# haliphinx/TCE-RVOS

Measured on AMD Instinct MI355X. Metric: clips/s (T=5, 360×640, Swin-T) at 1/2/4/8 MI355X; mask IoU vs ref, higher is better.
Workload: dtype f32 (3xf16-split MFMA, f32 accumulate); 1 GPU; swin_t_p4w7 T=5 360x640 + 32-token text, B=1 clip per forward, flags --with_box_refine --binary --f_token 8 --qtrans (BASELINE config 2); clips_in_flight_per_gpu=1, clips_per_forward=1, same_clip_in_group=False, ranks_per_gpu=1, parallelism=clip-sharded x1

## Files before the change

### include/tce_rvos_debug.h

```cpp
#ifndef TCE_RVOS_DEBUG_H
#define TCE_RVOS_DEBUG_H
#include <stdint.h>
#ifdef __cplusplus
extern "C" {
#endif
int tce_gemm_force_tile(int32_t tile);
int tce_debug_set_stamp_buffer(long long* dev_buf);
int tce_debug_set_epilogue(int32_t lds_staged);
int tce_debug_ffn_set_stamp_buffer(long long* dev_buf);
int tce_debug_ffn_set_half(int32_t mode);
int tce_debug_msda_set_lds(int32_t on);
int tce_debug_window_attn_set_mfma(int32_t on);
int tce_debug_mha_set_split(int32_t on);
int tce_debug_msda_set_fewq(int32_t on);
int tce_debug_conv3x3_set_waves(int32_t waves);
int tce_debug_conv3x3_set_pieces(int32_t pieces);
#ifdef __cplusplus
}
#endif
#endif
```

### tce-rvos_amd/_lib.py

```python
import ctypes as C
import os

HERE = os.path.dirname(os.path.abspath(__file__))
LIB_PATH = os.environ.get("TCE_LIB") or os.path.join(HERE, "lib", "libtce_rvos.so")

c_f = C.c_void_p
i32, i64, f32 = C.c_int32, C.c_int64, C.c_float


class GemmArgs(C.Structure):
    _fields_ = [("A", c_f), ("A2", c_f), ("W", c_f), ("bias", c_f), ("res", c_f), ("C", c_f),
                ("M", i32), ("N", i32), ("K", i32),
                ("lda", i32), ("lda2", i32), ("ldw", i32), ("ldc", i32), ("ldres", i32),
                ("act", i32), ("res_mode", i32), ("batch", i32),
                ("sA", i64), ("sA2", i64), ("sW", i64), ("sBias", i64), ("sC", i64), ("sRes", i64),
                ("conv", i32), ("T", i32), ("H", i32), ("Wd", i32), ("Cin", i32), ("Ho", i32), ("Wo", i32),
                ("kh", i32), ("kw", i32), ("stride", i32), ("pad", i32)]


class RowLinArgs(C.Structure):
    _fields_ = [("x", c_f), ("a2", c_f), ("packed", c_f), ("bias", c_f), ("res", c_f), ("out", c_f),
                ("g_in", c_f), ("be_in", c_f), ("g_out", c_f), ("be_out", c_f),
                ("ldx", i64), ("lda2", i64), ("ldres", i64), ("ldo", i64),
                ("sX", i64), ("sA2", i64), ("sRes", i64), ("sOut", i64),
# ... 67 lines not shown
    "tce_mha_ws_bytes": (i64, [i32, i32, i32]),
    "tce_mha_ws_f32": (i32, [c_f, c_f, c_f, c_f, c_f, i32, i32, i32, i32, i32, i32, i32, i32, i64, i64, i64, i64, c_f, f32, c_f]),
    "tce_ms_deform_attn_forward_f32": (i32, [c_f, c_f, c_f, c_f, c_f, c_f, i32, i32, i32, i32, i32, i32, i32, c_f]),
    "tce_ms_deform_attn_backward_f32": (i32, [c_f, c_f, c_f, c_f, c_f, c_f, c_f, c_f, c_f, i32, i32, i32, i32, i32, i32, i32, c_f]),
    "tce_msda_fused_f32": (i32, [c_f, c_f, c_f, c_f, C.POINTER(i32), i32, i32, i32, i32, i32, i32, i32, i32, c_f]),
    "tce_msda_fused_valid_f32": (i32, [c_f, c_f, c_f, c_f, C.POINTER(i32), C.POINTER(i32), i32, i32, i32, i32, i32, i32, i32,
                                       i32, c_f]),
    "tce_msda_fewq_raw_f32": (i32, [c_f, c_f, c_f, c_f, c_f, c_f, C.POINTER(i32), C.POINTER(i32), i32, i32, i32, i32, i32, i32, i32,
                                    i32, c_f]),
    "tce_contrastive_f32": (i32, [c_f, c_f, c_f, c_f, i32, i32, i32, i32, c_f]),
    "tce_pos_sine2d_f32": (i32, [c_f, c_f, i32, i32, i32, i32, c_f]),
    "tce_pos_sine2d_valid_f32": (i32, [c_f, c_f, i32, i32, i32, i32, i32, i32, c_f]),
    "tce_resize_nearest_f32": (i32, [c_f, c_f, c_f, i32, i32, i32, i32, i32, i32, c_f]),
    "tce_resize_bilinear_f32": (i32, [c_f, c_f, c_f, i32, i32, i32, i32, i32, i32, c_f]),
    "tce_resize_bilinear_ln_f32": (i32, [c_f, c_f, c_f, c_f, f32, c_f, i32, i32, i32, i32, i32, i32, c_f]),
    "tce_add_f32": (i32, [c_f, c_f, c_f, i64, i64, c_f]),
    "tce_tile_f32": (i32, [c_f, c_f, i64, i64, c_f]),
    "tce_sigmoid_f32": (i32, [c_f, c_f, i64, c_f]),
    "tce_copy_segments": (i32, [C.POINTER(CopySeg), i32, c_f]),
    "tce_box_refine_f32": (i32, [c_f, c_f, c_f, i32, i32, c_f]),
    "tce_mask_pack_f32": (i32, [c_f, c_f, c_f, i32, i32, i32, i32, c_f]),
    "tce_mask_tail_f32": (i32, [c_f, c_f, c_f, i32, c_f, i32, i32, i32, i32, i32, f32, f32, i32, c_f]),
    "tce_select_masks_u8": (i32, [c_f, c_f, c_f, c_f, i32, i32, i32, i32, i32, i32, i32, f32, c_f]),
    "tce_embed_ln_f32": (i32, [c_f, c_f, c_f, c_f, c_f, c_f, c_f, c_f, i32, i32, f32, i32, c_f]),
    "tce_mha_small64_f32": (i32, [c_f, c_f, i32, i32, f32, c_f]),
    "tce_mha_small64_seqs_f32": (i32, [c_f, i32, c_f, c_f, i32, i32, i32, f32, c_f]),
    "tce_embed_ln_seqs_f32": (i32, [c_f, c_f, c_f, c_f, c_f, c_f, c_f, i32, i32, i32, f32, i32, c_f]),
    "tce_mha_small64_lens_f32": (i32, [c_f, i32, c_f, c_f, i32, i32, i32, f32, c_f, c_f]),
    "tce_caption_lens_f32": (i32, [c_f, i32, i32, i32, i32, c_f, c_f, c_f, c_f]),
    "tce_tanh_f32": (i32, [c_f, c_f, i64, c_f]),
    "tce_ffn_packed_bytes": (i64, [i32, i32]),
    "tce_ffn_pack_f32": (i32, [c_f, c_f, c_f, c_f, i32, i32, c_f]),
    "tce_ffn_fused_f32": (i32, [c_f, i64, c_f, c_f, c_f, c_f, f32, c_f, c_f, f32, c_f, i64, i32, i32, i32, i32, c_f]),
    "tce_ffn_split_ws_floats": (i64, [i32, i32, i32, i32]),
    "tce_ffn_split_counters": (i32, [i32, i32, i32, i32]),
    "tce_ffn_set_wg_cap": (i32, [i32]),
    "tce_ffn_capped_grid": (i32, [i32, i32, i32, C.POINTER(i32)]),
    "tce_ffn_fused_split_f32": (i32, [c_f, i64, c_f, c_f, c_f, c_f, f32, c_f, c_f, f32, c_f, i64, i32, i32, i32, i32, c_f, i64, c_f, i32, c_f]),
    "tce_xattn_prepare_f32": (i32, [c_f, c_f, c_f, c_f, c_f, c_f, c_f, i32, i32, i32, c_f]),
    "tce_ffn_pack_batched_f32": (i32, [c_f, c_f, c_f, c_f, i32, i32, i32, c_f]),
    "tce_xattn_fused_f32": (i32, [C.POINTER(XattnArgs), c_f]),
    "tce_xattn_ffn_fused_f32": (i32, [C.POINTER(XattnArgs), C.POINTER(XattnFfnArgs), c_f]),
    "tce_ffn_pack_chain_f32": (i32, [c_f, c_f, c_f, c_f, i32, i32, c_f]),
    "tce_xattn_pack_f32": (i32, [c_f, c_f, c_f, c_f, c_f, i32, i32, i32, c_f]),
    "tce_xattn_prepare_lens_f32": (i32, [c_f, c_f, c_f, c_f, c_f, c_f, c_f, i32, i32, i32, c_f, c_f]),
    "tce_xattn_pack_lens_f32": (i32, [c_f, c_f, c_f, c_f, c_f, i32, i32, i32, c_f, c_f]),
    "tce_rowlin_packed_bytes": (i64, [i32, i32]),
    "tce_rowlin_pack_f32": (i32, [c_f, i64, c_f, i32, i32, c_f]),
    "tce_rowlin_f32": (i32, [C.POINTER(RowLinArgs), c_f]),
    "tce_conv3x3_packed_bytes": (i64, [i32, i32]),
    "tce_conv3x3_pack_f32": (i32, [c_f, c_f, i32, i32, c_f]),
    "tce_conv3x3_f32": (i32, [c_f, i64, c_f, c_f, c_f, i64, i32, i32, i32, i32, i32, c_f]),
    "tce_conv3x3_split_ws_floats": (i64, [i32, i32, i32]),
    "tce_conv3x3_split_pieces": (i32, [i32, i32, i32]),
    "tce_conv3x3_split_kstep": (i32, [i32, i32]),
    "tce_conv3x3_split_f32": (i32, [c_f, i64, c_f, c_f, c_f, i64, i32, i32, i32, i32, i32, c_f, i64, c_f]),
    "tce_fewrow_linear_f32": (i32, [C.POINTER(FewRowArgs), c_f]),
    "tce_thin_linear_splits": (i32, [i32, i32, i32]),
    "tce_thin_partials_f32": (i32, [c_f, i64, i32, c_f, i32, c_f, i64, c_f, i32, i32, i32, c_f]),
    "tce_splitk_reduce_f32": (i32, [c_f, i32, i32, i32, c_f, i32, c_f, i32, i32, c_f, i32, c_f, c_f, f32, c_f]),
    "tce_mha_small64_splits_f32": (i32, [c_f, i32, c_f, c_f, i32, i32, f32, c_f]),
    "tce_swin_attn_packed_bytes": (i64, [i32]),
    "tce_swin_attn_pack_f32": (i32, [c_f, c_f, c_f, i32, c_f]),
    "tce_swin_attn_fused_f32": (i32, [c_f, i64, c_f, c_f, c_f, c_f, c_f, c_f, f32, c_f, i64, i32, i32, i32, i32, i32, c_f]),
    "tce_graph_begin": (i32, [c_f]),
    "tce_graph_end": (i32, [c_f, C.POINTER(C.c_void_p)]),
    "tce_graph_launch": (i32, [C.c_void_p, c_f]),
    "tce_graph_destroy": (i32, [C.c_void_p]),
    "tce_graph_group": (i32, [C.POINTER(C.c_void_p), i32, C.POINTER(C.c_void_p)]),
}

DEBUG_SIGNATURES = {
    "tce_gemm_force_tile": (i32, [i32]),
    "tce_debug_set_stamp_buffer": (i32, [c_f]),
    "tce_debug_set_epilogue": (i32, [i32]),
    "tce_debug_ffn_set_stamp_buffer": (i32, [c_f]),
    "tce_debug_ffn_set_half": (i32, [i32]),
    "tce_debug_msda_set_lds": (i32, [i32]),
    "tce_debug_window_attn_set_mfma": (i32, [i32]),
    "tce_debug_mha_set_split": (i32, [i32]),
    "tce_debug_msda_set_fewq": (i32, [i32]),
    "tce_debug_conv3x3_set_waves": (i32, [i32]),
    "tce_debug_conv3x3_set_pieces": (i32, [i32]),
}

VIDEO_SIGNATURES = {
    "tce_label_objects_u8": (i32, [C.POINTER(LabelObj), i32, c_f, c_f, i32, i32, i32, i32, i32, i32, i32, f32, f32, c_f]),
}

A2D_GROUP_MAX = 16
EVAL_SIGNATURES = {
    "tce_a2d_masks_u8": (i32, [c_f, c_f, i32, i32, i32, i32, i32, i32, i32, f32, c_f]),
    "tce_rle_ws_bytes": (i64, [i32, i32, i32]),
    "tce_rle_counts_u32": (i32, [c_f, c_f, c_f, c_f, i32, i32, i32, c_f]),
    "tce_a2d_group_masks_u8": (i32, [C.POINTER(A2dGroupSample), i32, i32, i32, i32, f32, c_f]),
}

SCORE_SIGNATURES = {
    "tce_jf_ws_bytes": (i64, [i32, i32, i32, i32, i32]),
    "tce_jf_counts_i32": (i32, [c_f, c_f, c_f, c_f, i32, i32, i32, i32, i32, c_f]),
    "tce_rle_decode_ws_bytes": (i64, [i32, i32, i32, i32]),
    "tce_rle_decode_u8": (i32, [c_f, c_f, c_f, c_f, i32, i32, i32, i32, c_f]),
    "tce_mask_overlap_ws_bytes": (i64, [i32, i32, i32]),
    "tce_mask_overlap_i32": (i32, [c_f, c_f, c_f, c_f, i32, i32, i32, c_f]),
}

PNG_SIGNATURES = {
    "tce_png_stream_bound": (i64, [i32, i32, i32]),
    "tce_png_ws_bytes": (i64, [i32, i32, i32, i32]),
    "tce_png_deflate_u8": (i32, [c_f, c_f, c_f, c_f, i32, i32, i32, i32, i32, c_f]),
    "tce_png_deflate_dyn_u8": (i32, [c_f, c_f, c_f, c_f, i32, i32, i32, i32, i32, c_f]),
}

HEADERS = {"tce_rvos.h": SIGNATURES, "tce_rvos_debug.h": DEBUG_SIGNATURES, "tce_rvos_video.h": VIDEO_SIGNATURES,
           "tce_rvos_eval.h": EVAL_SIGNATURES, "tce_rvos_score.h": SCORE_SIGNATURES, "tce_rvos_png.h": PNG_SIGNATURES}

_LIB = None


class TceError(RuntimeError):
    pass


def lib():
    global _LIB
    if _LIB is None:
        if not os.path.exists(LIB_PATH):
            raise TceError(f"{LIB_PATH} not found: build the HIP extension first "
                           f"(python -c 'import __graft_entry__ as g; g.build()'); there is no fallback path")
        hwq = os.environ.get("GPU_MAX_HW_QUEUES")
        if hwq not in (None, "", "4"):
            import warnings
            warnings.warn(f"tce_rvos_amd: GPU_MAX_HW_QUEUES={hwq} is set; the HIP runtime's default (4) is the only value this "
                          f"launch program runs well with (1-3 crash the runtime, 5-16 double the clip time)", RuntimeWarning)
        l = C.CDLL(LIB_PATH)
        for name, (res, args) in [kv for table in HEADERS.values() for kv in table.items()]:
            fn = getattr(l, name)
            fn.restype, fn.argtypes = res, args
        _LIB = l
    return _LIB


def lib_raw():
    l = lib()
    return l.__dict__.get("_real", l)


def check(status, what=""):
    if status != 0:
        msg = lib().tce_last_error().decode(errors="replace")
        raise TceError(f"{what} failed ({status}): {msg}")
```

### tce-rvos_amd/csrc/rowlin.hip

```cpp
#include "common.h"
#include "gemm_epilogue.h"
#include "frag.h"
#include "tiles.h"
#include "../../include/tce_rvos.h"

namespace {

static __device__ long long* g_ffn_stamps = nullptr;

struct LinArgs {
  const float *x, *a2;
  const unsigned char* wpk;
  const float *bias, *res;
  float* out;
  const float *g_in, *be_in, *g_out, *be_out;
  long long ldx, lda2, ldres, ldo;
  long long sX, sA2, sRes, sOut;
  int M, N, a2_rows, act, res_mode;
  float eps_in, eps_out;
  int* range_flag;
  int single;
};

template <int K, bool ROW, bool SINGLE>
// ... 64 lines not shown
        fl[q] = *reinterpret_cast<const h16x8*>(st + (2 * q + 1) * PIECE);
      }
#pragma unroll
    for (int s = 0; s < KH; ++s) {
      if (s + 2 < KH) {
        fh[(s + 2) % 3] = *reinterpret_cast<const h16x8*>(st + (2 * s + 4) * PIECE);
        fl[(s + 2) % 3] = *reinterpret_cast<const h16x8*>(st + (2 * s + 5) * PIECE);
      }
      if (s < SLOTS) dma_half(s);
      __builtin_amdgcn_sched_barrier(0);
      if (!single) {
        acc = __builtin_amdgcn_mfma_f32_32x32x16_f16(fh[s % 3], xl[S0 + s], acc, 0, 0, 0);
        acc = __builtin_amdgcn_mfma_f32_32x32x16_f16(fl[s % 3], xh[S0 + s], acc, 0, 0, 0);
      }
      acc = __builtin_amdgcn_mfma_f32_32x32x16_f16(fh[s % 3], xh[S0 + s], acc, 0, 0, 0);
      __builtin_amdgcn_sched_barrier(0);
    }
    dma_next();
    cstage = cstage == 2 ? 0 : cstage + 1;
  };
  auto act_tile = [&](f32x16& acc) {
    if (p.act == 1) {
#pragma unroll
      for (int i = 0; i < 16; ++i) acc[i] = fmaxf(acc[i], 0.f);
    } else if (p.act == 2) {
#pragma unroll
      for (int i = 0; i < 16; ++i) acc[i] = tce_gelu(acc[i]);
    }
  };
  auto finish_tile = [&](f32x16& acc, const BiasTile& bt, const ResTile& rt) {
    const ResTile none = {};
    const BiasTile nob = {};
    if (p.res_mode == 0 || p.act != 0) {
      tile_bias_res<0>(acc, bt, none, wt, lane);
      act_tile(acc);
      if (p.res_mode == 1) tile_bias_res<1>(acc, nob, rt, wt, lane);
      else if (p.res_mode == 2) tile_bias_res<2>(acc, nob, rt, wt, lane);
    } else if (p.res_mode == 1) {
      tile_bias_res<1>(acc, bt, rt, wt, lane);
    } else {
      tile_bias_res<2>(acc, bt, rt, wt, lane);
    }
  };
  auto tile_mma = [&](f32x16& acc, const bool stores_follow) {
#pragma unroll
    for (int i = 0; i < 16; ++i) acc[i] = 0.f;
    half_mma(std::integral_constant<int, 0>{}, acc);
    asm volatile("s_waitcnt vmcnt(%0)" ::"n"(SLOTS) : "memory");
    __syncthreads();
    half_mma(std::integral_constant<int, 1>{}, acc);
    (void)stores_follow;
  };

  if (ROW) {
    f32x16 oacc[NTR];
#pragma unroll
    for (int t = 0; t < NTR; ++t) {
      tile_mma(oacc[t], false);
      asm volatile("s_waitcnt vmcnt(%0)" ::"n"(SLOTS) : "memory");
      __syncthreads();
    }
    {
      ResTile rt[NTR];
      if (p.res_mode != 0) {
#pragma unroll
        for (int t = 0; t < NTR; ++t) rt[t] = tile_res_load(res, p.ldres, m0, p.M, 32 * t, lane);
      }
#pragma unroll
      for (int t = 0; t < NTR; ++t) finish_tile(oacc[t], tile_bias_load(p.bias, 32 * t, lane), rt[t]);
    }
    if (p.g_out) rows_layernorm<NTR>(oacc, p.g_out, p.be_out, p.eps_out, hf);
#pragma unroll
    for (int t = 0; t < NTR; ++t) tile_store(oacc[t], out, p.ldo, m0, p.M, 32 * t, wt, lane, amax);
  } else {
    for (int t = t_begin; t < t_end; ++t) {
      ResTile rt = {};
      if (p.res_mode != 0) rt = tile_res_load(res, p.ldres, m0, p.M, 32 * t, lane);
      const BiasTile bt = tile_bias_load(p.bias, 32 * t, lane);
      f32x16 acc;
      tile_mma(acc, true);
      asm volatile("s_waitcnt vmcnt(%0)" ::"n"(SLOTS) : "memory");
      __syncthreads();
      finish_tile(acc, bt, rt);
      tile_store(acc, out, p.ldo, m0, p.M, 32 * t, wt, lane, amax);
    }
  }
  asm volatile("s_waitcnt vmcnt(0)" ::: "memory");
  tce_range_report(p.range_flag, amax);
  if (stamps) {
    stamps[2] = (long long)__builtin_amdgcn_s_memtime();
    stamps[3] = (long long)__builtin_amdgcn_s_memtime();
    stamps[5] = (long long)__builtin_amdgcn_s_memrealtime();
  }
}

__global__ void __launch_bounds__(256) rowlin_pack_kernel(const float* __restrict__ W, unsigned char* __restrict__ out,
                                                          const int N, const int K, const long long ldw,
                                                          const long long units, const int single) {
  const long long u = (long long)blockIdx.x * 256 + threadIdx.x;
  if (u >= units) return;
  const int KH = K / 32, HP = (2 * KH + 3) / 4 * 4;
  const int lane = (int)(u & 63);
  const long long pg = u >> 6;
  const int piece = (int)(pg % HP);
  const long long hb = pg / HP;
  const int t = (int)(hb >> 1), h = (int)(hb & 1);
  const int r = lane & 31, hf = lane >> 5, s = h * KH + (piece >> 1);
  u32x4 o = {0u, 0u, 0u, 0u};
  const int n = 32 * t + r;
  if (piece < 2 * KH && n < N) {
    float v[8];
#pragma unroll
    for (int j = 0; j < 8; ++j) v[j] = W[(long long)n * ldw + 16 * s + 8 * hf + j];
    const HL f = split8(v, single);
    o = __builtin_bit_cast(u32x4, (piece & 1) ? f.lo : f.hi);
  }
  reinterpret_cast<u32x4*>(out)[u] = o;
}

inline bool rowlin_shape_ok(int N, int K) {
  return (K == 96 || K == 128 || K == 192 || K == 256 || K == 384 || K == 512) && N > 0 && N % 32 == 0;
}
inline long long rowlin_units(int N, int K) {
  const int HP = (2 * (K / 32) + 3) / 4 * 4;
  return (long long)(2 * (N / 32) + 2) * HP * 64;
}

template <int K>
void rowlin_launch(const LinArgs& a, int batch, bool row, hipStream_t s) {
  const int rb = tce_cdiv(a.M, 128) * batch, ntiles = a.N / 32;
  int nz = 1;
  if (!row && K > 256) {
    nz = 256 / (rb > 0 ? rb : 1);
    if (nz > ntiles / 2) nz = ntiles / 2;
    if (nz < 1) nz = 1;
  } else if (!row) {
    while (nz < ntiles && rb * nz < 160 && ntiles / (nz * 2) >= 2) nz *= 2;
  }
  const dim3 grid(tce_cdiv(a.M, 128), batch, nz), block(256);
  if constexpr (K <= 384) {
    if (row) {
      if (a.single) hipLaunchKernelGGL((rowlin_kernel<K, true, true>), grid, block, 0, s, a);
      else hipLaunchKernelGGL((rowlin_kernel<K, true, false>), grid, block, 0, s, a);
      return;
    }
  }
  if (a.single) hipLaunchKernelGGL((rowlin_kernel<K, false, true>), grid, block, 0, s, a);
  else hipLaunchKernelGGL((rowlin_kernel<K, false, false>), grid, block, 0, s, a);
}

}

int tce_rowlin_set_stamps(long long* dev_buf) {
  return hipMemcpyToSymbol(HIP_SYMBOL(g_ffn_stamps), &dev_buf, sizeof(dev_buf)) == hipSuccess ? 0 : -1;
}

extern "C" int64_t tce_rowlin_packed_bytes(int32_t N, int32_t K) { return rowlin_shape_ok(N, K) ? rowlin_units(N, K) * 16 : -1; }

extern "C" int tce_rowlin_pack_f32(const float* W, int64_t ldw, void* packed, int32_t N, int32_t K, tceStream stream) {
  TCE_CHECK_ARG(rowlin_shape_ok(N, K), "tce_rowlin_pack_f32: unsupported shape N=%d K=%d (K in 96/128/192/256/384/512, N %% 32 == 0)", N, K);
  TCE_CHECK_ARG(W && packed && tce_aligned16(packed) && ldw >= K, "tce_rowlin_pack_f32: null / misaligned pointer or ldw < K");
  const long long units = rowlin_units(N, K);
  hipLaunchKernelGGL(rowlin_pack_kernel, dim3(tce_cdiv(units, 256)), dim3(256), 0, (hipStream_t)stream, W,
                     (unsigned char*)packed, N, K, (long long)ldw, units, tce_gemm_single_pass());
  TCE_CHECK_LAUNCH("tce_rowlin_pack_f32");
  return TCE_OK;
}

extern "C" int tce_rowlin_f32(const tceRowLinArgs* args, tceStream stream) {
  TCE_CHECK_ARG(args != nullptr, "tce_rowlin_f32: null args");
  const tceRowLinArgs& q = *args;
  TCE_CHECK_ARG(rowlin_shape_ok(q.N, q.K), "tce_rowlin_f32: unsupported shape N=%d K=%d", q.N, q.K);
  TCE_CHECK_ARG(q.M > 0 && q.x && q.packed && q.out, "tce_rowlin_f32: null pointer or M <= 0");
  TCE_CHECK_ARG(q.act >= 0 && q.act <= 2 && q.res_mode >= 0 && q.res_mode <= 2, "tce_rowlin_f32: bad act / res_mode");
  TCE_CHECK_ARG(q.res_mode == 0 || q.res, "tce_rowlin_f32: res_mode set without res");
  TCE_CHECK_ARG(q.ldx >= q.K && q.ldx % 4 == 0 && q.ldo >= q.N && q.ldo % 4 == 0 && (!q.res || (q.ldres >= q.N && q.ldres % 4 == 0)) &&
                    (!q.a2 || (q.lda2 >= q.K && q.lda2 % 4 == 0)),
                "tce_rowlin_f32: bad row pitch");
  TCE_CHECK_ARG(q.sX % 4 == 0 && q.sA2 % 4 == 0 && q.sRes % 4 == 0 && q.sOut % 4 == 0, "tce_rowlin_f32: batch strides must be multiples of 4 floats");
  TCE_CHECK_ARG(tce_aligned16(q.x) && tce_aligned16(q.out) && tce_aligned16(q.packed) && (!q.a2 || tce_aligned16(q.a2)) &&
                    (!q.res || tce_aligned16(q.res)) && (!q.bias || tce_aligned16(q.bias)),
                "tce_rowlin_f32: pointers must be 16-byte aligned");
  TCE_CHECK_ARG((!q.g_in || (q.be_in && tce_aligned16(q.g_in) && tce_aligned16(q.be_in))) &&
                    (!q.g_out || (q.be_out && tce_aligned16(q.g_out) && tce_aligned16(q.be_out))),
                "tce_rowlin_f32: LayerNorm gamma/beta must come in pairs, 16-byte aligned");
  TCE_CHECK_ARG(!q.g_out || (q.N == 256 && q.K <= 384), "tce_rowlin_f32: the output LayerNorm is built for N = 256, K <= 384");
  LinArgs a;
  a.x = q.x; a.a2 = q.a2; a.wpk = (const unsigned char*)q.packed; a.bias = q.bias; a.res = q.res; a.out = q.out;
  a.g_in = q.g_in; a.be_in = q.be_in; a.g_out = q.g_out; a.be_out = q.be_out;
  a.ldx = q.ldx; a.lda2 = q.lda2; a.ldres = q.ldres; a.ldo = q.ldo;
  a.sX = q.sX; a.sA2 = q.sA2; a.sRes = q.sRes; a.sOut = q.sOut;
  a.M = q.M; a.N = q.N; a.a2_rows = q.a2_rows; a.act = q.act; a.res_mode = q.res_mode;
  a.eps_in = q.eps_in; a.eps_out = q.eps_out; a.range_flag = tce_range_flag(); a.single = tce_gemm_single_pass();
  const int batch = q.batch > 0 ? q.batch : 1;
  const bool row = q.g_out != nullptr;
  hipStream_t s = (hipStream_t)stream;
  if (q.K == 512) rowlin_launch<512>(a, batch, row, s);
  else if (q.K == 384) rowlin_launch<384>(a, batch, row, s);
  else if (q.K == 256) rowlin_launch<256>(a, batch, row, s);
  else if (q.K == 192) rowlin_launch<192>(a, batch, row, s);
  else if (q.K == 128) rowlin_launch<128>(a, batch, row, s);
  else rowlin_launch<96>(a, batch, row, s);
  TCE_CHECK_LAUNCH("tce_rowlin_f32");
  return TCE_OK;
}
```

### tce-rvos_amd/ops.py

```python
import ctypes as C

import os
import threading

import torch

from ._lib import GemmArgs, check, lib

ACT_NONE, ACT_RELU, ACT_GELU, ACT_RELU_AFTER_RES = 0, 1, 2, 3
RES_NONE, RES_ADD, RES_MUL = 0, 1, 2


class Arena:

    ALIGN = 256
    FLAGS = 1 << 14

    def __init__(self, device, nbytes):
        self.device = torch.device(device)
        self.buf = torch.empty(int(nbytes), dtype=torch.uint8, device=self.device)
        self.off = 0
        self.peak = 0
        self.flags = torch.zeros(self.FLAGS, dtype=torch.int32, device=self.device)
        self.flag_off = 0
# ... 1170 lines not shown
            check(lib().tce_ffn_fused_split_f32(x.data_ptr(), ldx, packed.data_ptr(), b2.data_ptr(), gi, bi, eps_in, go, bo, eps_out,
                                                out.data_ptr(), ldo, M, Cn, Hd, act, ws.data_ptr(), ws.numel(), cnt.data_ptr(),
                                                cnt.numel(), _stream()), "tce_ffn_fused_split_f32")
            return
        check(lib().tce_ffn_fused_f32(x.data_ptr(), ldx, packed.data_ptr(), b2.data_ptr(), gi, bi, eps_in, go, bo, eps_out,
                                      out.data_ptr(), ldo, M, Cn, Hd, act, _stream()), "tce_ffn_fused_f32")
    if GEMM_PROFILE is None:
        go_()
        return out
    e0, e1 = torch.cuda.Event(enable_timing=True), torch.cuda.Event(enable_timing=True)
    e0.record()
    go_()
    e1.record()
    GEMM_PROFILE.append((f"ffn_fused_kernel<{Cn}", False, 4.0 * M * Cn * Hd, e0, e1))
    return out


class Routes:
    def __init__(self):
        self.rowlin = {}
        self.conv3 = {}
        self.keep = []

    def clear(self):
        self.rowlin.clear()
        self.conv3.clear()
        del self.keep[:]


DEFAULT_ROUTES = Routes()
_ROUTES = DEFAULT_ROUTES


class routes:

    def __init__(self, r):
        self.r, self.prev = r, None

    def __enter__(self):
        global _ROUTES
        self.prev, _ROUTES = _ROUTES, (self.r if self.r is not None else DEFAULT_ROUTES)
        return self

    def __exit__(self, *exc):
        global _ROUTES
        _ROUTES = self.prev
        return False


def current_routes():
    return _ROUTES


ROWLIN_MIN_ROWS = int(os.environ.get("TCE_ROWLIN_MIN_ROWS", 12000))
ROWLIN384_MAX_ROWS = int(os.environ.get("TCE_ROWLIN384_MAX_ROWS", 12000))
ROWLIN_K = (96, 128, 192, 256) + ((384,) if os.environ.get("TCE_ROWLIN_K384", "1") != "0" else ()) \
    + ((512,) if os.environ.get("TCE_ROWLIN_K512", "1") != "0" else ())


def rowlin_pack(w, N=None, K=None, ldw=None):
    _chk(w, "w")
    N = w.shape[0] if N is None else N
    K = w.shape[1] if K is None else K
    ldw = w.stride(0) if ldw is None else ldw
    nbytes = lib().tce_rowlin_packed_bytes(N, K)
    if nbytes < 0:
        raise ValueError(f"rowlin_pack: unsupported shape N={N} K={K}")
    out = torch.empty(nbytes, dtype=torch.uint8, device=w.device)
    check(lib().tce_rowlin_pack_f32(w.data_ptr(), ldw, out.data_ptr(), N, K, _stream()), "tce_rowlin_pack_f32")
    return out


def rowlin_register(w, table=None):
    if w.dim() != 2 or w.stride(1) != 1 or w.shape[1] not in ROWLIN_K or w.shape[0] % 32 or not w.is_cuda:
        return None
    r = _ROUTES if table is None else table
    key = (w.data_ptr(), w.shape[0], w.shape[1], w.stride(0), get_gemm_mode())
    if key not in r.rowlin:
        r.rowlin[key] = rowlin_pack(w)
        r.keep.append(w)
    return r.rowlin[key]


def rowlin(x, pk, out, M, N, K, ldx, ldo, bias=None, a2=None, lda2=0, a2_rows=0, act=ACT_NONE, res=None, ldres=0,
           res_mode=RES_NONE, ln_in=None, ln_out=None, eps_in=1e-5, eps_out=1e-5, batch=1, sX=0, sA2=0, sRes=0, sOut=0):
    from ._lib import RowLinArgs
    q = RowLinArgs()
    q.x, q.packed, q.out = x.data_ptr(), pk.data_ptr(), out.data_ptr()
    q.M, q.N, q.K, q.batch = M, N, K, batch
    q.ldx, q.ldo = ldx, ldo
    if a2 is not None:
        q.a2, q.lda2, q.a2_rows = a2.data_ptr(), lda2, a2_rows
    if bias is not None:
        q.bias = bias.data_ptr()
    if res_mode != RES_NONE:
        q.res, q.ldres = res.data_ptr(), ldres
    if ln_in is not None:
        q.g_in, q.be_in = ln_in[0].data_ptr(), ln_in[1].data_ptr()
    if ln_out is not None:
        q.g_out, q.be_out = ln_out[0].data_ptr(), ln_out[1].data_ptr()
    q.act, q.res_mode, q.eps_in, q.eps_out = act, res_mode, eps_in, eps_out
    q.sX, q.sA2, q.sRes, q.sOut = sX, sA2, sRes, sOut

    def go():
        check(lib().tce_rowlin_f32(C.byref(q), _stream()), "tce_rowlin_f32")
    if GEMM_PROFILE is None:
        go()
        return out
    e0, e1 = torch.cuda.Event(enable_timing=True), torch.cuda.Event(enable_timing=True)
    e0.record()
    go()
    e1.record()
    GEMM_PROFILE.append((f"rowlin_kernel<{K}", False, 2.0 * M * N * K * batch, e0, e1))
    return out


CONV3_MIN_PIXELS = int(os.environ.get("TCE_CONV3_MIN_PIXELS", 12000))
CONV3_SPLIT = os.environ.get("TCE_CONV3_SPLIT", "1") != "0"


def conv3x3_split_ws_floats(M, Cin=256, N=256):
    return int(lib().tce_conv3x3_split_ws_floats(M, Cin, N)) if CONV3_SPLIT else 0


def conv3x3_pack(w_cl, Cin):
    _chk(w_cl, "w")
    N = w_cl.shape[0]
    nbytes = lib().tce_conv3x3_packed_bytes(Cin, N)
    if nbytes < 0 or w_cl.shape[1] != 9 * Cin or not w_cl.is_contiguous():
        raise ValueError(f"conv3x3_pack: unsupported shape N={N} Cin={Cin}")
    out = torch.empty(nbytes, dtype=torch.uint8, device=w_cl.device)
    check(lib().tce_conv3x3_pack_f32(w_cl.data_ptr(), out.data_ptr(), Cin, N, _stream()), "tce_conv3x3_pack_f32")
    return out


def conv3x3_register(w_cl, Cin, table=None):
    if lib().tce_conv3x3_packed_bytes(Cin, w_cl.shape[0]) < 0 or w_cl.shape[1] != 9 * Cin:
        return None
    r = _ROUTES if table is None else table
    key = (w_cl.data_ptr(), w_cl.shape[0], w_cl.shape[1], get_gemm_mode())
    if key not in r.conv3:
        r.conv3[key] = conv3x3_pack(w_cl, Cin)
        r.keep.append(w_cl)
    return r.conv3[key]


def conv3x3(x, pk, T, H, W, Cin, N, bias=None, out=None, alloc=None):
    _chk(x, "x")
    M = T * H * W
    if out is None:
        out = alloc(M, N) if alloc else torch.empty(M, N, dtype=torch.float32, device=x.device)

    nws = conv3x3_split_ws_floats(M, Cin, N) if alloc else 0
    ws = alloc(nws) if nws else None

    def go():
        bp = bias.data_ptr() if bias is not None else None
        if ws is not None:
            check(lib().tce_conv3x3_split_f32(x.data_ptr(), x.stride(0), pk.data_ptr(), bp, out.data_ptr(), out.stride(0), T, H, W,
                                              Cin, N, ws.data_ptr(), nws, _stream()), "tce_conv3x3_split_f32")
        else:
            check(lib().tce_conv3x3_f32(x.data_ptr(), x.stride(0), pk.data_ptr(), bp, out.data_ptr(), out.stride(0), T, H, W, Cin,
                                        N, _stream()), "tce_conv3x3_f32")
    if GEMM_PROFILE is None:
        go()
        return out
    e0, e1 = torch.cuda.Event(enable_timing=True), torch.cuda.Event(enable_timing=True)
    e0.record()
    go()
# ... 123 lines not shown
```

Measured before the change: 179.8 clips/s.

## Add deep multi-stage LDS weight ring for rowlin kernels with K>=256

Adds a new rowlin kernel variant that streams packed weight pieces into a D-deep LDS ring via global-to-LDS DMA. It waits on vmcnt plus s_barrier instead of a full drain per tile, and stages bias/LN vectors and residual tiles through LDS. It is chosen automatically for K=256/384/512 using per-K depth tables, subject to grid-size and N limits. The packed weight buffer gains extra trailing padding so the deeper prefetch can run past the end, which costs more LDS per workgroup (occupancy 1) and adds complexity in vmcnt accounting.

```diff
diff --git a/include/tce_rvos_debug.h b/include/tce_rvos_debug.h
--- a/include/tce_rvos_debug.h
+++ b/include/tce_rvos_debug.h
@@ -15,6 +15,8 @@
 int tce_debug_msda_set_fewq(int32_t on);
 int tce_debug_conv3x3_set_waves(int32_t waves);
 int tce_debug_conv3x3_set_pieces(int32_t pieces);
+int tce_debug_rowlin_set_form(int32_t form);
+int tce_debug_rowlin_last_form(void);
 #ifdef __cplusplus
 }
 #endif
diff --git a/tce-rvos_amd/_lib.py b/tce-rvos_amd/_lib.py
--- a/tce-rvos_amd/_lib.py
+++ b/tce-rvos_amd/_lib.py
@@ -173,6 +173,8 @@
     "tce_debug_msda_set_fewq": (i32, [i32]),
     "tce_debug_conv3x3_set_waves": (i32, [i32]),
     "tce_debug_conv3x3_set_pieces": (i32, [i32]),
+    "tce_debug_rowlin_set_form": (i32, [i32]),
+    "tce_debug_rowlin_last_form": (i32, []),
 }
 
 VIDEO_SIGNATURES = {
diff --git a/tce-rvos_amd/csrc/rowlin.hip b/tce-rvos_amd/csrc/rowlin.hip
--- a/tce-rvos_amd/csrc/rowlin.hip
+++ b/tce-rvos_amd/csrc/rowlin.hip
@@ -170,6 +170,243 @@
       asm volatile("s_waitcnt vmcnt(%0)" ::"n"(SLOTS) : "memory");
       __syncthreads();
       finish_tile(acc, bt, rt);
+      tile_store(acc, out, p.ldo, m0, p.M, 32 * t, wt, lane, amax);
+    }
+  }
+  asm volatile("s_waitcnt vmcnt(0)" ::: "memory");
+  tce_range_report(p.range_flag, amax);
+  if (stamps) {
+    stamps[2] = (long long)__builtin_amdgcn_s_memtime();
+    stamps[3] = (long long)__builtin_amdgcn_s_memtime();
+    stamps[5] = (long long)__builtin_amdgcn_s_memrealtime();
+  }
+}
+
+typedef __attribute__((address_space(3))) unsigned char lds_u8;
+constexpr int DEEP_BIAS_CAP = 2048;
+
+template <int N>
+__device__ __forceinline__ void wait_vm_barrier() {
+  static_assert(N >= 0 && N < 64, "vmcnt is a 6-bit count");
+  asm volatile("s_waitcnt vmcnt(%0)\n\ts_barrier" ::"n"(N) : "memory");
+}
+
+template <int K, bool ROW, bool SINGLE, int D>
+__global__ void __launch_bounds__(256, 1) rowlin_deep_kernel(const LinArgs p) {
+  constexpr int WAVES = 4, KS = K / 16, KH = KS / 2;
+  constexpr int HP = (2 * KH + WAVES - 1) / WAVES * WAVES;
+  constexpr int SLOTS = HP / WAVES;
+  constexpr int HSTAGE = HP * PIECE;
+  constexpr int NTR = 8;
+  constexpr int WT0 = D * HSTAGE, VEC0 = WT0 + WAVES * WT_BYTES;
+  constexpr int VEC_BYTES = ROW ? 3 * PIECE : DEEP_BIAS_CAP * 4;
+  constexpr int AHEAD = SLOTS * (D - 2);
+  static_assert(KS % 2 == 0 && SLOTS <= KH && D >= 3, "piece count / ring depth");
+  static_assert(VEC0 + VEC_BYTES <= 160 * 1024, "LDS of one workgroup");
+  __shared__ __attribute__((aligned(16))) unsigned char smem[VEC0 + VEC_BYTES];
+
+  const int tid = threadIdx.x, lane = tid & 63;
+  const int wave = __builtin_amdgcn_readfirstlane(tid >> 6);
+  const int hf = lane >> 5;
+  const int bz = blockIdx.y;
+  const int m0 = blockIdx.x * (32 * WAVES) + wave * 32;
+  if (p.M < 0) {
+    reinterpret_cast<u32x4*>(smem)[tid] = u32x4{0u, 0u, 0u, 0u};
+    reinterpret_cast<u32x4*>(smem + VEC0)[tid & 127] = u32x4{0u, 0u, 0u, 0u};
+  }
+
+  const float* const x = p.x + bz * p.sX;
+  const float* const a2 = p.a2 ? p.a2 + bz * p.sA2 : nullptr;
+  const float* const res = p.res ? p.res + bz * p.sRes : nullptr;
+  float* const out = p.out + bz * p.sOut;
+  const int ntiles = p.N / 32;
+  const int t_begin = ROW ? 0 : (int)((long long)blockIdx.z * ntiles / gridDim.z);
+  const int t_end = ROW ? ntiles : (int)((long long)(blockIdx.z + 1) * ntiles / gridDim.z);
+
+  long long* const stamps = (g_ffn_stamps && blockIdx.x < 1024 && bz == 0 && blockIdx.z == 0 && tid == 0) ? g_ffn_stamps + blockIdx.x * 8 : nullptr;
+  if (stamps) {
+    stamps[0] = (long long)__builtin_amdgcn_s_memtime();
+    stamps[4] = (long long)__builtin_amdgcn_s_memrealtime();
+  }
+  const unsigned voff = lane * 16;
+  const unsigned ring0 = (unsigned)(unsigned long long)(lds_u8*)smem;
+  float* const vec = reinterpret_cast<float*>(smem + VEC0);
+  if (ROW) {
+    const float* const src = wave == 0 ? p.bias : wave == 1 ? p.g_out : wave == 2 ? p.be_out : nullptr;
+    if (src) glds16(reinterpret_cast<const unsigned char*>(src), voff, ring0 + VEC0 + wave * PIECE);
+    else if (wave == 0) reinterpret_cast<f32x4*>(vec)[lane] = f32x4{0.f, 0.f, 0.f, 0.f};
+  } else {
+#pragma unroll
+    for (int j = 0; j < DEEP_BIAS_CAP / 256 / WAVES; ++j) {
+      const int c = wave + WAVES * j;
+      if (p.bias) glds16(reinterpret_cast<const unsigned char*>(p.bias), (unsigned)min(c * 256 + lane * 4, p.N - 4) * 4u, ring0 + VEC0 + c * PIECE);
+      else reinterpret_cast<f32x4*>(vec)[c * 64 + lane] = f32x4{0.f, 0.f, 0.f, 0.f};
+    }
+  }
+  const unsigned char* wp = p.wpk + ((long long)2 * t_begin * HP + wave) * PIECE;
+  const unsigned wbase = ring0 + wave * PIECE;
+  int dstage = 0;
+  auto dma_half = [&](int q) { glds16(wp + (long long)q * WAVES * PIECE, voff, wbase + (unsigned)(dstage * HSTAGE + q * WAVES * PIECE)); };
+  auto dma_next = [&]() {
+    wp += HP * PIECE;
+    dstage = dstage == D - 1 ? 0 : dstage + 1;
+  };
+#pragma unroll
+  for (int h = 0; h < D - 1; ++h) {
+#pragma unroll
+    for (int q = 0; q < SLOTS; ++q) dma_half(q);
+    dma_next();
+  }
+
+  float* const wt = reinterpret_cast<float*>(smem + WT0 + wave * WT_BYTES);
+  const unsigned wt_lds = (unsigned)(unsigned long long)(lds_u8*)wt;
+  h16x8 xh[KS], xl[KS];
+  load_x_frags<K>(x, p.ldx, a2, p.lda2, p.a2_rows, m0, p.M, wt, lane, p.g_in, p.be_in, p.eps_in, xh, xl, SINGLE);
+  constexpr int single = SINGLE;
+  tce_amax_t amax = 0;
+  if (stamps) stamps[6] = (long long)__builtin_amdgcn_s_memtime();
+  asm volatile("s_waitcnt vmcnt(0) lgkmcnt(0)\n\ts_barrier" ::: "memory");
+  if (stamps) stamps[1] = (long long)__builtin_amdgcn_s_memtime();
+
+  int cstage = 0;
+  auto half_mma = [&](auto half_c, f32x16& acc) {
+    constexpr int S0 = decltype(half_c)::value * KH;
+    const unsigned char* const st = smem + cstage * HSTAGE + lane * 16;
+    h16x8 fh[3], fl[3];
+#pragma unroll
+    for (int q = 0; q < 2; ++q)
+      if (q < KH) {
+        fh[q] = *reinterpret_cast<const h16x8*>(st + (2 * q) * PIECE);
+        fl[q] = *reinterpret_cast<const h16x8*>(st + (2 * q + 1) * PIECE);
+      }
+#pragma unroll
+    for (int s = 0; s < KH; ++s) {
+      __builtin_amdgcn_sched_barrier(0);
+      if (!single) {
+        acc = __builtin_amdgcn_mfma_f32_32x32x16_f16(fh[s % 3], xl[S0 + s], acc, 0, 0, 0);
+        __builtin_amdgcn_sched_barrier(0);
+        if (s + 2 < KH) fh[(s + 2) % 3] = *reinterpret_cast<const h16x8*>(st + (2 * s + 4) * PIECE);
+        __builtin_amdgcn_sched_barrier(0);
+        acc = __builtin_amdgcn_mfma_f32_32x32x16_f16(fl[s % 3], xh[S0 + s], acc, 0, 0, 0);
+        __builtin_amdgcn_sched_barrier(0);
+        if (s + 2 < KH) fl[(s + 2) % 3] = *reinterpret_cast<const h16x8*>(st + (2 * s + 5) * PIECE);
+        __builtin_amdgcn_sched_barrier(0);
+      }
+      acc = __builtin_amdgcn_mfma_f32_32x32x16_f16(fh[s % 3], xh[S0 + s], acc, 0, 0, 0);
+      __builtin_amdgcn_sched_barrier(0);
+      if (single && s + 2 < KH) fh[(s + 2) % 3] = *reinterpret_cast<const h16x8*>(st + (2 * s + 4) * PIECE);
+      if (s < SLOTS) dma_half(s);
+      __builtin_amdgcn_sched_barrier(0);
+    }
+    dma_next();
+    cstage = cstage == D - 1 ? 0 : cstage + 1;
+  };
+  auto act_tile = [&](f32x16& acc) {
+    if (p.act == 1) {
+#pragma unroll
+      for (int i = 0; i < 16; ++i) acc[i] = fmaxf(acc[i], 0.f);
+    } else if (p.act == 2) {
+#pragma unroll
+      for (int i = 0; i < 16; ++i) acc[i] = tce_gelu(acc[i]);
+    }
+  };
+
+  if (ROW) {
+    f32x16 oacc[NTR];
+#pragma unroll
+    for (int t = 0; t < NTR; ++t) {
+#pragma unroll
+      for (int i = 0; i < 16; ++i) oacc[t][i] = 0.f;
+      half_mma(std::integral_constant<int, 0>{}, oacc[t]);
+      wait_vm_barrier<AHEAD>();
+      half_mma(std::integral_constant<int, 1>{}, oacc[t]);
+      wait_vm_barrier<AHEAD>();
+    }
+    const ResTile none = {};
+    const BiasTile nob = {};
+    {
+      ResTile rt[NTR];
+      if (p.res_mode != 0) {
+#pragma unroll
+        for (int t = 0; t < NTR; ++t) rt[t] = tile_res_load(res, p.ldres, m0, p.M, 32 * t, lane);
+      }
+#pragma unroll
+      for (int t = 0; t < NTR; ++t) {
+        const BiasTile bt = tile_bias_load(vec, 32 * t, lane);
+        if (p.res_mode == 0 || p.act != 0) {
+          tile_bias_res<0>(oacc[t], bt, none, wt, lane);
+          act_tile(oacc[t]);
+          if (p.res_mode == 1) tile_bias_res<1>(oacc[t], nob, rt[t], wt, lane);
+          else if (p.res_mode == 2) tile_bias_res<2>(oacc[t], nob, rt[t], wt, lane);
+        } else if (p.res_mode == 1) {
+          tile_bias_res<1>(oacc[t], bt, rt[t], wt, lane);
+        } else {
+          tile_bias_res<2>(oacc[t], bt, rt[t], wt, lane);
+        }
+      }
+    }
+    rows_layernorm<NTR>(oacc, vec + 256, vec + 512, p.eps_out, hf);
+#pragma unroll
+    for (int t = 0; t < NTR; ++t) tile_store(oacc[t], out, p.ldo, m0, p.M, 32 * t, wt, lane, amax);
+  } else {
+    const bool has_res = p.res_mode != 0;
+    const int r = lane & 31, cr = lane >> 3;
+    const int row0 = min(m0, p.M - 1);
+    const unsigned char* rbase = has_res ? reinterpret_cast<const unsigned char*>(res + (long long)row0 * p.ldres + 32 * t_begin) : nullptr;
+    unsigned roff[4];
+#pragma unroll
+    for (int i = 0; i < 4; ++i) {
+      const int rr = 8 * i + cr;
+      roff[i] = (unsigned)(((long long)(min(m0 + rr, p.M - 1) - row0) * p.ldres + 4 * ((lane & 7) ^ ((rr >> 1) & 7))) * 4);
+    }
+    const unsigned char* const rimg = reinterpret_cast<const unsigned char*>(wt) + r * 128;
+    const int rsw = (r >> 1) & 7;
+    for (int t = t_begin; t < t_end; ++t) {
+      if (has_res) {
+#pragma unroll
+        for (int i = 0; i < 4; ++i) glds16(rbase, roff[i], wt_lds + i * PIECE);
+        rbase += 128;
+      }
+      f32x16 acc;
+#pragma unroll
+      for (int i = 0; i < 16; ++i) acc[i] = 0.f;
+      half_mma(std::integral_constant<int, 0>{}, acc);
+      if (has_res) wait_vm_barrier<AHEAD + 4>();
+      else wait_vm_barrier<AHEAD>();
+      half_mma(std::integral_constant<int, 1>{}, acc);
+      if (has_res) wait_vm_barrier<(D == 3 ? 1 : 2) * SLOTS>();
+      else wait_vm_barrier<AHEAD>();
+      const BiasTile bt = tile_bias_load(vec, 32 * t, lane);
+      const BiasTile nob = {};
+      f32x4 rv[4];
+      if (has_res) {
+#pragma unroll
+        for (int g = 0; g < 4; ++g) rv[g] = *reinterpret_cast<const f32x4*>(rimg + 16 * ((2 * g + hf) ^ rsw));
+      }
+      auto bias_res = [&](auto res_c, const BiasTile& b) {
+        constexpr int RES = decltype(res_c)::value;
+#pragma unroll
+        for (int g = 0; g < 4; ++g) {
+          const f32x4 bv = b.v[g];
+#pragma unroll
+          for (int c = 0; c < 4; ++c) {
+            if (RES == 1) acc[4 * g + c] = acc[4 * g + c] + bv[c] + rv[g][c];
+            else if (RES == 2) acc[4 * g + c] = (acc[4 * g + c] + bv[c]) * rv[g][c];
+            else acc[4 * g + c] += bv[c];
+          }
+        }
+      };
+      if (p.res_mode == 0 || p.act != 0) {
+        bias_res(std::integral_constant<int, 0>{}, bt);
+        act_tile(acc);
+        if (p.res_mode == 1) bias_res(std::integral_constant<int, 1>{}, nob);
+        else if (p.res_mode == 2) bias_res(std::integral_constant<int, 2>{}, nob);
+      } else if (p.res_mode == 1) {
+        bias_res(std::integral_constant<int, 1>{}, bt);
+      } else {
+        bias_res(std::integral_constant<int, 2>{}, bt);
+      }
+      __builtin_amdgcn_wave_barrier();
       tile_store(acc, out, p.ldo, m0, p.M, 32 * t, wt, lane, amax);
     }
   }
@@ -209,9 +446,32 @@
 inline bool rowlin_shape_ok(int N, int K) {
   return (K == 96 || K == 128 || K == 192 || K == 256 || K == 384 || K == 512) && N > 0 && N % 32 == 0;
 }
+constexpr int ROWLIN_TRAIL = 7;
 inline long long rowlin_units(int N, int K) {
   const int HP = (2 * (K / 32) + 3) / 4 * 4;
-  return (long long)(2 * (N / 32) + 2) * HP * 64;
+  return (long long)(2 * (N / 32) + ROWLIN_TRAIL) * HP * 64;
+}
+
+static int g_rowlin_form = 0;
+static int g_rowlin_last = 0;
+
+template <int K> struct DeepDepths { static constexpr int a = 0, b = 0, c = 0, stream = 0, row = 0; };
+template <> struct DeepDepths<256> { static constexpr int a = 3, b = 5, c = 8, stream = 0, row = 3; };
+template <> struct DeepDepths<384> { static constexpr int a = 3, b = 4, c = 5, stream = 4, row = 3; };
+template <> struct DeepDepths<512> { static constexpr int a = 3, b = 4, c = 0, stream = 4, row = 0; };
+
+template <int K, int D>
+void rowlin_deep_launch(const LinArgs& a, bool row, dim3 grid, hipStream_t s) {
+  const dim3 block(256);
+  if constexpr (K <= 384) {
+    if (row) {
+      if (a.single) hipLaunchKernelGGL((rowlin_deep_kernel<K, true, true, D>), grid, block, 0, s, a);
+      else hipLaunchKernelGGL((rowlin_deep_kernel<K, true, false, D>), grid, block, 0, s, a);
+      return;
+    }
+  }
+  if (a.single) hipLaunchKernelGGL((rowlin_deep_kernel<K, false, true, D>), grid, block, 0, s, a);
+  else hipLaunchKernelGGL((rowlin_deep_kernel<K, false, false, D>), grid, block, 0, s, a);
 }
 
 template <int K>
@@ -226,6 +486,20 @@
     while (nz < ntiles && rb * nz < 160 && ntiles / (nz * 2) >= 2) nz *= 2;
   }
   const dim3 grid(tce_cdiv(a.M, 128), batch, nz), block(256);
+  g_rowlin_last = 1;
+  if constexpr (K >= 256) {
+    using DD = DeepDepths<K>;
+    const bool eligible = row || (a.N <= DEEP_BIAS_CAP && (K > 256 || (long long)grid.x * grid.y * grid.z <= tce_cu_count()));
+    const int f = g_rowlin_form;
+    const int d = (f == DD::a || f == DD::b || (f == DD::c && f != 0)) ? f : (row ? DD::row : DD::stream);
+    if (eligible && f != 1 && d != 0) {
+      if (d == DD::a) rowlin_deep_launch<K, DD::a>(a, row, grid, s);
+      else if (d == DD::b) rowlin_deep_launch<K, DD::b>(a, row, grid, s);
+      else if constexpr (DD::c != 0) rowlin_deep_launch<K, DD::c>(a, row, grid, s);
+      g_rowlin_last = d;
+      return;
+    }
+  }
   if constexpr (K <= 384) {
     if (row) {
       if (a.single) hipLaunchKernelGGL((rowlin_kernel<K, true, true>), grid, block, 0, s, a);
@@ -242,6 +516,15 @@
 int tce_rowlin_set_stamps(long long* dev_buf) {
   return hipMemcpyToSymbol(HIP_SYMBOL(g_ffn_stamps), &dev_buf, sizeof(dev_buf)) == hipSuccess ? 0 : -1;
 }
+
+extern "C" int tce_debug_rowlin_set_form(int32_t form) {
+  TCE_CHECK_ARG(form == 0 || form == 1 || (form >= 3 && form <= ROWLIN_TRAIL + 1),
+                "tce_debug_rowlin_set_form: 0 (automatic), 1 (three-stage ring under __syncthreads) or a ring depth 3..8");
+  g_rowlin_form = form;
+  return TCE_OK;
+}
+
+extern "C" int tce_debug_rowlin_last_form(void) { return g_rowlin_last; }
 
 extern "C" int64_t tce_rowlin_packed_bytes(int32_t N, int32_t K) { return rowlin_shape_ok(N, K) ? rowlin_units(N, K) * 16 : -1; }
 
diff --git a/tce-rvos_amd/ops.py b/tce-rvos_amd/ops.py
--- a/tce-rvos_amd/ops.py
+++ b/tce-rvos_amd/ops.py
@@ -1276,9 +1276,22 @@
     return r.rowlin[key]
 
 
+_ROWLIN_FORM = int(os.environ.get("TCE_ROWLIN_FORM", 0))
+_rowlin_form_applied = False
+
+
+def _apply_rowlin_form():
+    global _rowlin_form_applied
+    if not _rowlin_form_applied:
+        _rowlin_form_applied = True
+        if _ROWLIN_FORM:
+            check(lib().tce_debug_rowlin_set_form(_ROWLIN_FORM), "tce_debug_rowlin_set_form")
+
+
 def rowlin(x, pk, out, M, N, K, ldx, ldo, bias=None, a2=None, lda2=0, a2_rows=0, act=ACT_NONE, res=None, ldres=0,
            res_mode=RES_NONE, ln_in=None, ln_out=None, eps_in=1e-5, eps_out=1e-5, batch=1, sX=0, sA2=0, sRes=0, sOut=0):
     from ._lib import RowLinArgs
+    _apply_rowlin_form()
     q = RowLinArgs()
     q.x, q.packed, q.out = x.data_ptr(), pk.data_ptr(), out.data_ptr()
     q.M, q.N, q.K, q.batch = M, N, K, batch
```

Measured after the change: 179.4 clips/s, median of 2. About the same (-0.2%).
